# ablab/spades

Measured on NVIDIA H100. Metric: Mk-mers/s (extract+count+index) k=55, 150 bp reads, higher is better.
Workload: dtype u64

## Files before the change

spades_b200/csrc/mphf.cu:

```cuda
#include <math.h>

#include <algorithm>

#include "mphf_dev.cuh"

namespace sg {

template <int NW>
__global__ void mphf_insert_k(KeyTable t, const uint64_t *__restrict__ alive, uint64_t n, int level, MphfDev m, uint64_t level_start,
                              uint64_t *__restrict__ coll) {
    uint64_t i = (uint64_t)blockIdx.x * blockDim.x + threadIdx.x;
    if (i >= n) return;
    const int64_t ki = alive ? (int64_t)alive[i] : (int64_t)i;
    Kmer<NW> k = table_key<NW>(t, ki);
    const uint32_t b = kmer_bucket<NW>(k, m.B);
    uint64_t w;
    const uint64_t pos = level_pos<NW>(m, k, b, level, &w);
    const unsigned long long bit = 1ull << (pos & 63);
    unsigned long long old = atomicOr((unsigned long long *)&m.bits[w], bit);
    if (old & bit) atomicOr((unsigned long long *)&coll[w - level_start], bit);
}

__global__ void mphf_clear_k(uint64_t *__restrict__ bits, uint64_t *__restrict__ coll, uint64_t nwords) {
    uint64_t i = (uint64_t)blockIdx.x * blockDim.x + threadIdx.x;
    if (i >= nwords) return;
    uint64_t c = coll[i];
    if (c) { bits[i] &= ~c; coll[i] = 0; }
}

template <int NW>
__global__ void mphf_filter_k(KeyTable t, const uint64_t *__restrict__ alive, uint64_t n, int level, MphfDev m, uint64_t *__restrict__ next,
                              uint64_t cap, unsigned long long *__restrict__ next_n) {
    uint64_t i = (uint64_t)blockIdx.x * blockDim.x + threadIdx.x;
    bool keep = false;
    int64_t ki = 0;
    if (i < n) {
        ki = alive ? (int64_t)alive[i] : (int64_t)i;
        Kmer<NW> k = table_key<NW>(t, ki);
        const uint32_t b = kmer_bucket<NW>(k, m.B);
        uint64_t w;
        const uint64_t pos = level_pos<NW>(m, k, b, level, &w);
        keep = !((m.bits[w] >> (pos & 63)) & 1ull);
    }
    __shared__ unsigned s_warp[8];
    __shared__ unsigned long long s_base;
    const unsigned mask = __ballot_sync(0xffffffffu, keep);
    const int lane = threadIdx.x & 31, warp = threadIdx.x >> 5;
    if (lane == 0) s_warp[warp] = __popc(mask);
    __syncthreads();
    if (threadIdx.x == 0) {
        unsigned tot = 0;
        for (int w = 0; w < 8; ++w) { unsigned c = s_warp[w]; s_warp[w] = tot; tot += c; }
        s_base = tot ? atomicAdd(next_n, (unsigned long long)tot) : 0ull;
    }
    __syncthreads();
    if (keep) {
        const uint64_t slot = s_base + s_warp[warp] + __popc(mask & ((1u << lane) - 1));
        if (slot < cap) next[slot] = (uint64_t)ki;
    }
}

template <int NW>
__global__ void mphf_advance_k(KeyTable t, const uint64_t *__restrict__ alive, uint64_t n, int level, MphfDev m, uint64_t *__restrict__ next,
                               uint64_t cap, unsigned long long *__restrict__ next_n, int do_insert, uint64_t next_level_start,
                               uint64_t *__restrict__ coll) {
    uint64_t i = (uint64_t)blockIdx.x * blockDim.x + threadIdx.x;
    bool keep = false;
    int64_t ki = 0;
    if (i < n) {
        ki = alive ? (int64_t)alive[i] : (int64_t)i;
        Kmer<NW> k = table_key<NW>(t, ki);
        const uint32_t b = kmer_bucket<NW>(k, m.B);
        LevelHasher lh(xxh3_128<NW>(k));
        uint64_t h = 0;
        for (int l = 0; l <= level; ++l) h = lh.next();
        size_t p = (size_t)level * m.B + b;
        uint64_t pos = mulhi64(h, m.dom[p]);
        keep = !((m.bits[m.woff[p] + (pos >> 6)] >> (pos & 63)) & 1ull);
        if (keep && do_insert) {
            h = lh.next();
            p += m.B;
            pos = mulhi64(h, m.dom[p]);
            const uint64_t w = m.woff[p] + (pos >> 6);
            const unsigned long long bit = 1ull << (pos & 63);
            unsigned long long old = atomicOr((unsigned long long *)&m.bits[w], bit);
            if (old & bit) atomicOr((unsigned long long *)&coll[w - next_level_start], bit);
        }
    }
    __shared__ unsigned s_warp[8];
    __shared__ unsigned long long s_base;
    const unsigned mask = __ballot_sync(0xffffffffu, keep);
    const int lane = threadIdx.x & 31, warp = threadIdx.x >> 5;
    if (lane == 0) s_warp[warp] = __popc(mask);
    __syncthreads();
    if (threadIdx.x == 0) {
        unsigned tot = 0;
        for (int w = 0; w < 8; ++w) { unsigned c = s_warp[w]; s_warp[w] = tot; tot += c; }
        s_base = tot ? atomicAdd(next_n, (unsigned long long)tot) : 0ull;
    }
    __syncthreads();
    if (keep) {
        const uint64_t slot = s_base + s_warp[warp] + __popc(mask & ((1u << lane) - 1));
        if (slot < cap) next[slot] = (uint64_t)ki;
    }
}

__global__ void mphf_blockpop_k(const uint64_t *__restrict__ bits, uint64_t nblocks, uint32_t *__restrict__ pop) {
    uint64_t i = (uint64_t)blockIdx.x * blockDim.x + threadIdx.x;
    if (i >= nblocks) return;
    const ulonglong2 *p = reinterpret_cast<const ulonglong2 *>(bits + i * 8);
    uint32_t s = 0;
#pragma unroll
    for (int q = 0; q < 4; ++q) { ulonglong2 v = p[q]; s += __popcll(v.x) + __popcll(v.y); }
    pop[i] = s;
}

__global__ void mphf_piecebase_k(const uint64_t *__restrict__ gscan, const uint64_t *__restrict__ woff, uint32_t B, uint64_t total_blocks,
                                 uint64_t *__restrict__ piece_base, uint64_t *__restrict__ lastrank) {
    uint32_t b = blockIdx.x * blockDim.x + threadIdx.x;
    if (b >= B) return;
    uint64_t run = 0;
    for (int l = 0; l < kLevels; ++l) {
        const size_t p = (size_t)l * B + b;
        const uint64_t blk0 = woff[p] >> 3;
        const uint64_t blk1 = (p + 1 < (size_t)kLevels * B) ? (woff[p + 1] >> 3) : total_blocks;
        piece_base[p] = run;
        run += gscan[blk1] - gscan[blk0];
    }
    lastrank[b] = run;
}
__global__ void mphf_ranks_k(const uint64_t *__restrict__ gscan, const uint64_t *__restrict__ woff, const uint64_t *__restrict__ piece_base,
                             uint32_t npieces, uint64_t nblocks, uint64_t *__restrict__ ranks) {
    uint64_t i = (uint64_t)blockIdx.x * blockDim.x + threadIdx.x;
    if (i >= nblocks) return;
    uint32_t lo = 0, hi = npieces - 1;
    while (lo < hi) {
        uint32_t mid = (lo + hi + 1) >> 1;
        if ((woff[mid] >> 3) <= i) lo = mid; else hi = mid - 1;
    }
    ranks[i] = piece_base[lo] + gscan[i] - gscan[woff[lo] >> 3];
}

template <int NW>
__global__ void mphf_lookup_k(MphfDev m, const uint64_t *__restrict__ keys, uint64_t n, uint64_t *__restrict__ out) {
    uint64_t i = (uint64_t)blockIdx.x * blockDim.x + threadIdx.x;
    if (i >= n) return;
    Kmer<NW> k;
#pragma unroll
    for (int q = 0; q < NW; ++q) k.w[q] = keys[i * NW + q];
    out[i] = mphf_lookup_dev<NW>(m, k);
}

MphfDev mphf_dev(const Mphf *m) {
    MphfDev d;
    d.dom = m->d_dom.p; d.woff = m->d_woff.p; d.starts = m->d_starts.p; d.bits = m->bits.p; d.ranks = m->ranks.p; d.B = (uint32_t)m->B;
    return d;
}

template <int NW>
static void build_nw(Ctx *ctx, const KSet *ks, Mphf *m) {
    cudaStream_t st = ctx->stream;
    const int B = ks->B;
    const uint64_t n = (uint64_t)ks->n;
    m->dom.assign((size_t)kLevels * B, 0); m->nchar.assign((size_t)kLevels * B, 0); m->woff.assign((size_t)kLevels * B + 1, 0);
    std::vector<uint64_t> level_start(kLevels + 1, 0);
    {
        uint64_t off = 0;
        std::vector<double> pcol(B);
        std::vector<uint64_t> hd(B);
        for (int b = 0; b < B; ++b) {
            uint64_t nb = (uint64_t)ks->bsz[b];
            double gamma = 4.0;
            hd[b] = (uint64_t)ceil((double)nb * gamma);
            pcol[b] = nb ? 1.0 - pow(((gamma * (double)nb - 1) / (gamma * (double)nb)), (double)(nb - 1)) : 0.0;
        }
        for (int l = 0; l < kLevels; ++l) {
            level_start[l] = off;
            for (int b = 0; b < B; ++b) {
                const size_t p = (size_t)l * B + b;
                m->woff[p] = off;
                if (ks->bsz[b] == 0) { m->dom[p] = 64; m->nchar[p] = 0; continue; }
                uint64_t d = (((uint64_t)((double)hd[b] * pow(pcol[b], l)) + 63) / 64) * 64;
                if (d == 0) d = 64;
                m->dom[p] = d;
                m->nchar[p] = 1 + d / 64;
                off += ((m->nchar[p] + 7) / 8) * 8;
            }
        }
        level_start[kLevels] = off;
        m->woff[(size_t)kLevels * B] = off;
        m->total_words = off;
    }
    m->starts.assign(B + 1, 0);
    for (int b = 0; b < B; ++b) m->starts[b + 1] = (uint64_t)ks->bsz[b];
    for (int i = 1; i < B; ++i) m->starts[i] += m->starts[i - 1];
    m->bsz = ks->bsz;
    m->lastrank.assign(B, 0);
    const uint64_t total_words = m->total_words;
    const uint64_t nblocks = total_words / 8;
    m->bits.alloc(ctx, total_words + 8, true);
    m->ranks.alloc(ctx, nblocks + 1, true);
    m->d_dom.alloc(ctx, m->dom.size(), true); m->d_woff.alloc(ctx, m->woff.size(), true); m->d_starts.alloc(ctx, m->starts.size(), true);
    SG_CUDA(cudaMemsetAsync(m->bits.p, 0, m->bits.bytes(), st));
    SG_CUDA(cudaMemcpyAsync(m->d_dom.p, m->dom.data(), m->dom.size() * 8, cudaMemcpyHostToDevice, st));
    SG_CUDA(cudaMemcpyAsync(m->d_woff.p, m->woff.data(), m->woff.size() * 8, cudaMemcpyHostToDevice, st));
    SG_CUDA(cudaMemcpyAsync(m->d_starts.p, m->starts.data(), m->starts.size() * 8, cudaMemcpyHostToDevice, st));
    if (n == 0 || total_words == 0) { SG_CUDA(cudaStreamSynchronize(st)); return; }

    MphfDev md = mphf_dev(m);
    const uint64_t l0_words = level_start[1] - level_start[0];
    DArr<uint64_t> coll(ctx, l0_words + 8);
    SG_CUDA(cudaMemsetAsync(coll.p, 0, coll.bytes(), st));
    DArr<unsigned long long> d_cnt(ctx, 1);
    DArr<uint64_t> aliveA, aliveB;
    auto place = [&](const KeyTable &t, uint64_t n, int b_lo, int b_hi) {
        auto clear = [&](int l) {
            const uint64_t w0 = m->woff[(size_t)l * B + b_lo], nw = m->woff[(size_t)l * B + b_hi] - w0;
            mphf_clear_k<<<div_up((int64_t)nw, 256), 256, 0, st>>>(m->bits.p + w0, coll.p + (w0 - level_start[l]), nw);
            ctx->launches++;
        };
        const uint64_t *alive = nullptr;
        uint64_t n_alive = n;
        mphf_insert_k<NW><<<div_up((int64_t)n_alive, 256), 256, 0, st>>>(t, alive, n_alive, 0, md, level_start[0], coll.p);
        ctx->launches++;
        clear(0);
        for (int l = 0; l < kLevels - 1 && n_alive; ++l) {
            const bool last = (l == kLevels - 2);
            DArr<uint64_t> &next = (l & 1) ? aliveA : aliveB;
            uint64_t cap = (l == 0) ? n_alive / 2 + 1024 : n_alive;
            if (next.n < cap) next.alloc(ctx, cap);
            SG_CUDA(cudaMemsetAsync(d_cnt.p, 0, 8, st));
            mphf_advance_k<NW><<<div_up((int64_t)n_alive, 256), 256, 0, st>>>(t, alive, n_alive, l, md, next.p, (uint64_t)next.n, d_cnt.p,
                                                                             last ? 0 : 1, last ? 0 : level_start[l + 1], coll.p);
            ctx->launches++;
            if (!last) clear(l + 1);
            SG_CUDA(cudaGetLastError());
            unsigned long long c = 0;
            SG_CUDA(cudaMemcpyAsync(&c, d_cnt.p, 8, cudaMemcpyDeviceToHost, st));
            SG_CUDA(cudaStreamSynchronize(st));
            SG_CHECK(c <= next.n, 6, "internal: MPHF survivor list overflow");
            alive = next.p;
            n_alive = c;
        }
        SG_CHECK(n_alive == 0, 7, "MPHF: keys fell through all 24 bitset levels (reference would use its order-dependent fallback map); unsupported");
    };
    if (!ks->on_host) {
        place(make_table(ks), n, 0, B);
    } else {
        ChunkStager stage(ks, false);
        for (size_t c = 0; c < ks->chunks.size(); ++c) {
            const Chunk &ch = ks->chunks[c];
            const uint64_t *keys = nullptr;
            stage.acquire(c, &keys, nullptr);
            if (ch.n) {
                KeyTable t;
                t.nchunks = 1; t.first[0] = 0; t.first[1] = ch.n; t.keys[0] = keys;
                place(t, (uint64_t)ch.n, ch.b_lo, ch.b_hi);
            }
            stage.release(c);
        }
    }
    DArr<uint32_t> pop(ctx, nblocks + 1);
    DArr<uint64_t> gscan(ctx, nblocks + 1), piece_base(ctx, (size_t)kLevels * B), d_last(ctx, B);
    SG_CUDA(cudaMemsetAsync(pop.p + nblocks, 0, 4, st));
    mphf_blockpop_k<<<div_up((int64_t)nblocks, 256), 256, 0, st>>>(m->bits.p, nblocks, pop.p);
    ctx->launches++;
    exclusive_scan_u32_to_u64(ctx, pop.p, gscan.p, nblocks + 1);
    mphf_piecebase_k<<<div_up(B, 128), 128, 0, st>>>(gscan.p, m->d_woff.p, (uint32_t)B, nblocks, piece_base.p, d_last.p);
    mphf_ranks_k<<<div_up((int64_t)nblocks, 256), 256, 0, st>>>(gscan.p, m->d_woff.p, piece_base.p, (uint32_t)(kLevels * B), nblocks, m->ranks.p);
    ctx->launches += 2;
    SG_CUDA(cudaGetLastError());
    SG_CUDA(cudaMemcpyAsync(m->lastrank.data(), d_last.p, (size_t)B * 8, cudaMemcpyDeviceToHost, st));
    SG_CUDA(cudaStreamSynchronize(st));
    for (int b = 0; b < B; ++b) SG_CHECK(m->lastrank[b] == (uint64_t)ks->bsz[b], 6, "internal: MPHF is not minimal (rank total != bucket size)");
}

Mphf *mphf_build(Ctx *ctx, const KSet *ks) {
    Mphf *m = new Mphf();
    m->ctx = ctx; m->K = ks->K; m->nw = ks->nw; m->B = ks->B; m->n = ks->n;
    ctx->times.stage_h2d_bytes = 0;
    cudaEvent_t a, b;
    cudaEventCreate(&a); cudaEventCreate(&b);
    cudaEventRecord(a, ctx->stream);
    try {
        switch (ks->nw) {
            case 1: build_nw<1>(ctx, ks, m); break;
            case 2: build_nw<2>(ctx, ks, m); break;
            case 3: build_nw<3>(ctx, ks, m); break;
            default: build_nw<4>(ctx, ks, m); break;
        }
    } catch (...) { cudaEventDestroy(a); cudaEventDestroy(b); delete m; throw; }
    cudaEventRecord(b, ctx->stream);
    cudaEventSynchronize(b);
    float ms = 0; cudaEventElapsedTime(&ms, a, b);
    ctx->times.mphf += ms;
    cudaEventDestroy(a); cudaEventDestroy(b);
    return m;
}

struct SerPiece { uint64_t src_word; uint64_t dst_byte; uint64_t nwords; uint32_t from_ranks; uint32_t pad; };
struct SerPatch { uint64_t dst_byte; uint64_t value; uint32_t nbytes; uint32_t pad; };

__global__ void ser_pieces_k(const SerPiece *__restrict__ pieces, const uint64_t *__restrict__ bits, const uint64_t *__restrict__ ranks,
                             uint32_t *__restrict__ img32) {
    const SerPiece p = pieces[blockIdx.x];
    const uint64_t *src = (p.from_ranks ? ranks : bits) + p.src_word;
    uint32_t *dst = img32 + (p.dst_byte >> 2);
    for (uint64_t i = threadIdx.x; i < p.nwords; i += blockDim.x) {
        const uint64_t v = src[i];
        dst[2 * i] = (uint32_t)v;
        dst[2 * i + 1] = (uint32_t)(v >> 32);
    }
}
__global__ void ser_patches_k(const SerPatch *__restrict__ patches, uint64_t n, uint32_t *__restrict__ img32) {
    uint64_t i = (uint64_t)blockIdx.x * blockDim.x + threadIdx.x;
    if (i >= n) return;
    const SerPatch p = patches[i];
    img32[p.dst_byte >> 2] = (uint32_t)p.value;
    if (p.nbytes == 8) img32[(p.dst_byte >> 2) + 1] = (uint32_t)(p.value >> 32);
}

size_t mphf_serialized_size(const Mphf *m) {
    const int B = m->B;
    size_t total = 8;
    for (int b = 0; b < B; ++b) {
        total += 28 + 8;
        if (m->bsz[b])
            for (int l = 0; l < kLevels; ++l) {
                const size_t p = (size_t)l * B + b;
                total += 16 + 8 * m->nchar[p] + 8 + 8 * ((m->nchar[p] + 7) / 8);
            }
    }
    return total + 8 * ((size_t)B + 1);
}

void mphf_serialize_to(const Mphf *m, uint8_t *out, size_t cap) {
    Ctx *ctx = m->ctx;
    const int B = m->B;
    const size_t total = mphf_serialized_size(m);
    SG_CHECK(total <= cap, 2, "output buffer too small for the serialized index");
    std::vector<SerPiece> pieces;
    std::vector<SerPatch> patches;
    size_t pos = 0;
    auto patch = [&](uint64_t v, uint32_t nbytes) { patches.push_back(SerPatch{pos, v, nbytes, 0}); pos += nbytes; };
// ... 57 lines not shown
```

spades_b200/csrc/mphf_dev.cuh:

```cuda
#pragma once
#include "sgpu_internal.h"

namespace sg {

struct KeyTable {
    int nchunks;
    int64_t first[kMaxChunks + 1];
    const uint64_t *keys[kMaxChunks];
};

template <int NW>
__device__ __forceinline__ Kmer<NW> table_key(const KeyTable &t, int64_t i) {
    int c = 0, hi = t.nchunks - 1;
    while (c < hi) {
        const int mid = (c + hi + 1) >> 1;
        if (t.first[mid] <= i) c = mid; else hi = mid - 1;
    }
    const uint64_t *p = t.keys[c] + (i - t.first[c]) * NW;
    Kmer<NW> k;
#pragma unroll
    for (int q = 0; q < NW; ++q) k.w[q] = p[q];
    return k;
}

struct MphfDev {
    const uint64_t *dom;
    const uint64_t *woff;
    const uint64_t *starts;
    uint64_t *bits;
    const uint64_t *ranks;
    uint32_t B;
};

template <int NW>
__device__ __forceinline__ uint64_t level_pos(const MphfDev &m, const Kmer<NW> &k, uint32_t b, int level, uint64_t *word_index) {
    LevelHasher lh(xxh3_128<NW>(k));
    uint64_t h = 0;
    for (int l = 0; l <= level; ++l) h = lh.next();
    const uint64_t pos = mulhi64(h, m.dom[(size_t)level * m.B + b]);
    *word_index = m.woff[(size_t)level * m.B + b] + (pos >> 6);
    return pos;
}

template <int NW>
__device__ __forceinline__ uint64_t mphf_lookup_dev(const MphfDev &m, const Kmer<NW> &k) {
    const uint32_t b = kmer_bucket<NW>(k, m.B);
    LevelHasher lh(xxh3_128<NW>(k));
    for (int l = 0; l < kLevels - 1; ++l) {
        const uint64_t h = lh.next();
        const size_t p = (size_t)l * m.B + b;
        const uint64_t pos = mulhi64(h, m.dom[p]);
        const uint64_t wbase = m.woff[p];
        const uint64_t wi = pos >> 6;
        const uint64_t word = m.bits[wbase + wi];
        if ((word >> (pos & 63)) & 1ull) {
            uint64_t r = m.ranks[(wbase >> 3) + (pos >> 9)];
            for (uint64_t w = (pos >> 9) << 3; w < wi; ++w) r += __popcll(m.bits[wbase + w]);
            r += __popcll(word & ((1ull << (pos & 63)) - 1));
            return m.starts[b] + r;
        }
    }
    return ~0ull;
}


MphfDev mphf_dev(const Mphf *m);

inline KeyTable make_table(const KSet *ks) {
    SG_CHECK((int)ks->chunks.size() <= kMaxChunks, 6, "too many result chunks for the key table");
    KeyTable t;
    t.nchunks = (int)ks->chunks.size();
    for (int c = 0; c < t.nchunks; ++c) { t.first[c] = ks->chunks[c].first; t.keys[c] = ks->chunks[c].keys.p; }
    t.first[t.nchunks] = ks->n;
    if (t.nchunks == 0) { t.nchunks = 1; t.first[0] = 0; t.first[1] = 0; t.keys[0] = nullptr; }
    return t;
}

}
```

Before: 8693.

## Carry hasher state for surviving keys across MPHF levels instead of rehashing

The MPHF placement no longer reloads each surviving k-mer and recomputes xxh3 and the level-hash chain at every level. It now stores the hasher state (s0, s1) and the bucket id in survivor arrays and resumes from there. Bucket ids come from a binary search over the sorted bucket boundaries instead of rehashing, keys are read with streaming vectorized loads, and each thread handles four items in a grid-stride loop. Placement is also split into bucket ranges sized to the free device memory. In exchange, more bytes are written per survivor and the code is considerably more complex.

```diff
diff --git a/spades_b200/csrc/mphf.cu b/spades_b200/csrc/mphf.cu
--- a/spades_b200/csrc/mphf.cu
+++ b/spades_b200/csrc/mphf.cu
@@ -6,19 +6,198 @@
 
 namespace sg {
 
+static const int kPlaceThreads = 256, kPlaceU = 4, kPlaceTile = kPlaceThreads * kPlaceU, kPlaceCtasPerSm = 4;
 template <int NW>
-__global__ void mphf_insert_k(KeyTable t, const uint64_t *__restrict__ alive, uint64_t n, int level, MphfDev m, uint64_t level_start,
-                              uint64_t *__restrict__ coll) {
-    uint64_t i = (uint64_t)blockIdx.x * blockDim.x + threadIdx.x;
-    if (i >= n) return;
-    const int64_t ki = alive ? (int64_t)alive[i] : (int64_t)i;
-    Kmer<NW> k = table_key<NW>(t, ki);
-    const uint32_t b = kmer_bucket<NW>(k, m.B);
-    uint64_t w;
-    const uint64_t pos = level_pos<NW>(m, k, b, level, &w);
-    const unsigned long long bit = 1ull << (pos & 63);
-    unsigned long long old = atomicOr((unsigned long long *)&m.bits[w], bit);
-    if (old & bit) atomicOr((unsigned long long *)&coll[w - level_start], bit);
+constexpr int test0_ctas_per_sm() { return NW >= 4 ? 2 : NW >= 2 ? 3 : kPlaceCtasPerSm; }
+
+struct PlaceRange {
+    const uint64_t *bnd;
+    uint64_t base;
+    uint32_t b_lo, b_hi;
+};
+
+__device__ __forceinline__ uint32_t bucket_at(const uint64_t *__restrict__ bnd, uint32_t lo, uint32_t hi, uint64_t g) {
+    while (lo < hi) {
+        const uint32_t mid = (lo + hi + 1) >> 1;
+        if (__ldg(bnd + mid) <= g) lo = mid; else hi = mid - 1;
+    }
+    return lo;
+}
+
+template <int NW>
+__device__ __forceinline__ Kmer<NW> load_key_stream(const uint64_t *__restrict__ keys, uint64_t i) {
+    Kmer<NW> k;
+    const uint64_t *p = keys + i * NW;
+    if (NW % 2 == 0) {
+#pragma unroll
+        for (int q = 0; q < NW; q += 2) { const ulonglong2 v = __ldcs(reinterpret_cast<const ulonglong2 *>(p + q)); k.w[q] = v.x; k.w[q + 1] = v.y; }
+    } else {
+#pragma unroll
+        for (int q = 0; q < NW; ++q) k.w[q] = __ldcs(p + q);
+    }
+    return k;
+}
+
+__device__ __forceinline__ void level_insert(const MphfDev &m, const size_t (&p)[kPlaceU], const uint64_t (&h)[kPlaceU], unsigned todo,
+                                             uint64_t level_start, uint64_t *__restrict__ coll) {
+    uint64_t w[kPlaceU];
+    unsigned long long bit[kPlaceU], old[kPlaceU];
+#pragma unroll
+    for (int j = 0; j < kPlaceU; ++j) {
+        w[j] = 0; bit[j] = 0; old[j] = 0;
+        if ((todo >> j) & 1u) {
+            const uint64_t pos = mulhi64(h[j], __ldg(m.dom + p[j]));
+            w[j] = __ldg(m.woff + p[j]) + (pos >> 6);
+            bit[j] = 1ull << (pos & 63);
+            old[j] = atomicOr((unsigned long long *)&m.bits[w[j]], bit[j]);
+        }
+    }
+#pragma unroll
+    for (int j = 0; j < kPlaceU; ++j)
+        if (old[j] & bit[j]) atomicOr((unsigned long long *)&coll[w[j] - level_start], bit[j]);
+}
+
+__device__ __forceinline__ bool level_bit(const MphfDev &m, size_t p, uint64_t h) {
+    const uint64_t pos = mulhi64(h, __ldg(m.dom + p));
+    return (m.bits[__ldg(m.woff + p) + (pos >> 6)] >> (pos & 63)) & 1ull;
+}
+
+struct LevelStates {
+    uint64_t *s0, *s1;
+    uint32_t *b;
+};
+
+__device__ __forceinline__ void tile_buckets(const PlaceRange &r, uint64_t t0, uint64_t t1, uint32_t *lo, uint32_t *hi) {
+    *lo = bucket_at(r.bnd, r.b_lo, r.b_hi - 1, r.base + t0);
+    *hi = bucket_at(r.bnd, *lo, r.b_hi - 1, r.base + t1 - 1);
+}
+
+__device__ __forceinline__ void append_states(const uint64_t (&s0)[kPlaceU], const uint64_t (&s1)[kPlaceU], const uint32_t (&b)[kPlaceU], unsigned keep,
+                                              LevelStates out, uint64_t cap, unsigned long long *__restrict__ out_n) {
+    __shared__ unsigned s_warp[kPlaceThreads / 32];
+    __shared__ unsigned long long s_base;
+    const int lane = threadIdx.x & 31, warp = threadIdx.x >> 5;
+    const unsigned c = __popc(keep);
+    unsigned incl = c;
+#pragma unroll
+    for (int d = 1; d < 32; d <<= 1) { const unsigned v = __shfl_up_sync(0xffffffffu, incl, d); if (lane >= d) incl += v; }
+    if (lane == 31) s_warp[warp] = incl;
+    __syncthreads();
+    if (threadIdx.x == 0) {
+        unsigned tot = 0;
+#pragma unroll
+        for (int w = 0; w < kPlaceThreads / 32; ++w) { const unsigned v = s_warp[w]; s_warp[w] = tot; tot += v; }
+        s_base = tot ? atomicAdd(out_n, (unsigned long long)tot) : 0ull;
+    }
+    __syncthreads();
+    uint64_t slot = s_base + s_warp[warp] + (incl - c);
+#pragma unroll
+    for (int j = 0; j < kPlaceU; ++j)
+        if ((keep >> j) & 1u) {
+            if (slot < cap) { out.s0[slot] = s0[j]; out.s1[slot] = s1[j]; out.b[slot] = b[j]; }
+            ++slot;
+        }
+}
+
+template <int NW>
+__global__ void __launch_bounds__(kPlaceThreads, kPlaceCtasPerSm) mphf_insert0_k(const uint64_t *__restrict__ keys, uint64_t n, PlaceRange r, MphfDev m,
+                                                                uint64_t level_start, uint64_t *__restrict__ coll) {
+    for (uint64_t t0 = (uint64_t)blockIdx.x * kPlaceTile; t0 < n; t0 += (uint64_t)gridDim.x * kPlaceTile) {
+        const uint64_t t1 = min(t0 + (uint64_t)kPlaceTile, n);
+        uint32_t blo, bhi;
+        tile_buckets(r, t0, t1, &blo, &bhi);
+        Kmer<NW> k[kPlaceU];
+#pragma unroll
+        for (int j = 0; j < kPlaceU; ++j) {
+            const uint64_t i = t0 + (uint64_t)j * kPlaceThreads + threadIdx.x;
+            if (i < t1) k[j] = load_key_stream<NW>(keys, i);
+        }
+        size_t p[kPlaceU];
+        uint64_t h[kPlaceU];
+        unsigned todo = 0;
+#pragma unroll
+        for (int j = 0; j < kPlaceU; ++j) {
+            const uint64_t i = t0 + (uint64_t)j * kPlaceThreads + threadIdx.x;
+            p[j] = 0; h[j] = 0;
+            if (i < t1) { p[j] = bucket_at(r.bnd, blo, bhi, r.base + i); h[j] = xxh3_128<NW>(k[j]).hi; todo |= 1u << j; }
+        }
+        level_insert(m, p, h, todo, level_start, coll);
+    }
+}
+
+template <int NW>
+__global__ void __launch_bounds__(kPlaceThreads, test0_ctas_per_sm<NW>()) mphf_test0_k(const uint64_t *__restrict__ keys, uint64_t n, PlaceRange r, MphfDev m,
+                                                              LevelStates out, uint64_t cap, unsigned long long *__restrict__ out_n,
+                                                              uint64_t next_level_start, uint64_t *__restrict__ coll) {
+    for (uint64_t t0 = (uint64_t)blockIdx.x * kPlaceTile; t0 < n; t0 += (uint64_t)gridDim.x * kPlaceTile) {
+        const uint64_t t1 = min(t0 + (uint64_t)kPlaceTile, n);
+        uint32_t blo, bhi;
+        tile_buckets(r, t0, t1, &blo, &bhi);
+        Kmer<NW> k[kPlaceU];
+#pragma unroll
+        for (int j = 0; j < kPlaceU; ++j) {
+            const uint64_t i = t0 + (uint64_t)j * kPlaceThreads + threadIdx.x;
+            if (i < t1) k[j] = load_key_stream<NW>(keys, i);
+        }
+        uint64_t s0[kPlaceU], s1[kPlaceU];
+        uint32_t b[kPlaceU];
+        bool set[kPlaceU];
+#pragma unroll
+        for (int j = 0; j < kPlaceU; ++j) {
+            const uint64_t i = t0 + (uint64_t)j * kPlaceThreads + threadIdx.x;
+            set[j] = true;
+            if (i < t1) {
+                const Hash128 h = xxh3_128<NW>(k[j]);
+                s0[j] = h.hi; s1[j] = h.lo;
+                b[j] = bucket_at(r.bnd, blo, bhi, r.base + i);
+                set[j] = level_bit(m, b[j], s0[j]);
+            }
+        }
+        unsigned keep = 0;
+        size_t p[kPlaceU];
+#pragma unroll
+        for (int j = 0; j < kPlaceU; ++j) {
+            keep |= (set[j] ? 0u : 1u) << j;
+            p[j] = (size_t)m.B + b[j];
+        }
+        level_insert(m, p, s1, keep, next_level_start, coll);
+        append_states(s0, s1, b, keep, out, cap, out_n);
+    }
+}
+
+__global__ void __launch_bounds__(kPlaceThreads, kPlaceCtasPerSm) mphf_advance_k(LevelStates in, uint64_t n, int level, MphfDev m, LevelStates out, uint64_t cap,
+                                                                unsigned long long *__restrict__ out_n, int do_insert, uint64_t next_level_start,
+                                                                uint64_t *__restrict__ coll) {
+    for (uint64_t t0 = (uint64_t)blockIdx.x * kPlaceTile; t0 < n; t0 += (uint64_t)gridDim.x * kPlaceTile) {
+        const uint64_t t1 = min(t0 + (uint64_t)kPlaceTile, n);
+        uint64_t s0[kPlaceU], s1[kPlaceU];
+        uint32_t b[kPlaceU];
+#pragma unroll
+        for (int j = 0; j < kPlaceU; ++j) {
+            const uint64_t i = t0 + (uint64_t)j * kPlaceThreads + threadIdx.x;
+            if (i < t1) { s0[j] = __ldcs(in.s0 + i); s1[j] = __ldcs(in.s1 + i); b[j] = __ldcs(in.b + i); }
+        }
+        unsigned keep = 0;
+        size_t p[kPlaceU];
+        uint64_t h1[kPlaceU];
+#pragma unroll
+        for (int j = 0; j < kPlaceU; ++j) {
+            const uint64_t i = t0 + (uint64_t)j * kPlaceThreads + threadIdx.x;
+            p[j] = (size_t)(level + 1) * m.B + b[j]; h1[j] = 0;
+            if (i < t1) {
+                LevelHasher lh(Hash128{s1[j], s0[j]});
+                lh.level = level;
+                const uint64_t h = lh.next();
+                if (!level_bit(m, (size_t)level * m.B + b[j], h)) {
+                    keep |= 1u << j;
+                    s0[j] = lh.s0; s1[j] = lh.s1;
+                    h1[j] = lh.next();
+                }
+            }
+        }
+        if (do_insert) level_insert(m, p, h1, keep, next_level_start, coll);
+        append_states(s0, s1, b, keep, out, cap, out_n);
+    }
 }
 
 __global__ void mphf_clear_k(uint64_t *__restrict__ bits, uint64_t *__restrict__ coll, uint64_t nwords) {
@@ -26,83 +205,6 @@
     if (i >= nwords) return;
     uint64_t c = coll[i];
     if (c) { bits[i] &= ~c; coll[i] = 0; }
-}
-
-template <int NW>
-__global__ void mphf_filter_k(KeyTable t, const uint64_t *__restrict__ alive, uint64_t n, int level, MphfDev m, uint64_t *__restrict__ next,
-                              uint64_t cap, unsigned long long *__restrict__ next_n) {
-    uint64_t i = (uint64_t)blockIdx.x * blockDim.x + threadIdx.x;
-    bool keep = false;
-    int64_t ki = 0;
-    if (i < n) {
-        ki = alive ? (int64_t)alive[i] : (int64_t)i;
-        Kmer<NW> k = table_key<NW>(t, ki);
-        const uint32_t b = kmer_bucket<NW>(k, m.B);
-        uint64_t w;
-        const uint64_t pos = level_pos<NW>(m, k, b, level, &w);
-        keep = !((m.bits[w] >> (pos & 63)) & 1ull);
-    }
-    __shared__ unsigned s_warp[8];
-    __shared__ unsigned long long s_base;
-    const unsigned mask = __ballot_sync(0xffffffffu, keep);
-    const int lane = threadIdx.x & 31, warp = threadIdx.x >> 5;
-    if (lane == 0) s_warp[warp] = __popc(mask);
-    __syncthreads();
-    if (threadIdx.x == 0) {
-        unsigned tot = 0;
-        for (int w = 0; w < 8; ++w) { unsigned c = s_warp[w]; s_warp[w] = tot; tot += c; }
-        s_base = tot ? atomicAdd(next_n, (unsigned long long)tot) : 0ull;
-    }
-    __syncthreads();
-    if (keep) {
-        const uint64_t slot = s_base + s_warp[warp] + __popc(mask & ((1u << lane) - 1));
-        if (slot < cap) next[slot] = (uint64_t)ki;
-    }
-}
-
-template <int NW>
-__global__ void mphf_advance_k(KeyTable t, const uint64_t *__restrict__ alive, uint64_t n, int level, MphfDev m, uint64_t *__restrict__ next,
-                               uint64_t cap, unsigned long long *__restrict__ next_n, int do_insert, uint64_t next_level_start,
-                               uint64_t *__restrict__ coll) {
-    uint64_t i = (uint64_t)blockIdx.x * blockDim.x + threadIdx.x;
-    bool keep = false;
-    int64_t ki = 0;
-    if (i < n) {
-        ki = alive ? (int64_t)alive[i] : (int64_t)i;
-        Kmer<NW> k = table_key<NW>(t, ki);
-        const uint32_t b = kmer_bucket<NW>(k, m.B);
-        LevelHasher lh(xxh3_128<NW>(k));
-        uint64_t h = 0;
-        for (int l = 0; l <= level; ++l) h = lh.next();
-        size_t p = (size_t)level * m.B + b;
-        uint64_t pos = mulhi64(h, m.dom[p]);
-        keep = !((m.bits[m.woff[p] + (pos >> 6)] >> (pos & 63)) & 1ull);
-        if (keep && do_insert) {
-            h = lh.next();
-            p += m.B;
-            pos = mulhi64(h, m.dom[p]);
-            const uint64_t w = m.woff[p] + (pos >> 6);
-            const unsigned long long bit = 1ull << (pos & 63);
-            unsigned long long old = atomicOr((unsigned long long *)&m.bits[w], bit);
-            if (old & bit) atomicOr((unsigned long long *)&coll[w - next_level_start], bit);
-        }
-    }
-    __shared__ unsigned s_warp[8];
-    __shared__ unsigned long long s_base;
-    const unsigned mask = __ballot_sync(0xffffffffu, keep);
-    const int lane = threadIdx.x & 31, warp = threadIdx.x >> 5;
-    if (lane == 0) s_warp[warp] = __popc(mask);
-    __syncthreads();
-    if (threadIdx.x == 0) {
-        unsigned tot = 0;
-        for (int w = 0; w < 8; ++w) { unsigned c = s_warp[w]; s_warp[w] = tot; tot += c; }
-        s_base = tot ? atomicAdd(next_n, (unsigned long long)tot) : 0ull;
-    }
-    __syncthreads();
-    if (keep) {
-        const uint64_t slot = s_base + s_warp[warp] + __popc(mask & ((1u << lane) - 1));
-        if (slot < cap) next[slot] = (uint64_t)ki;
-    }
 }
 
 __global__ void mphf_blockpop_k(const uint64_t *__restrict__ bits, uint64_t nblocks, uint32_t *__restrict__ pop) {
@@ -208,55 +310,90 @@
     if (n == 0 || total_words == 0) { SG_CUDA(cudaStreamSynchronize(st)); return; }
 
     MphfDev md = mphf_dev(m);
-    const uint64_t l0_words = level_start[1] - level_start[0];
-    DArr<uint64_t> coll(ctx, l0_words + 8);
-    SG_CUDA(cudaMemsetAsync(coll.p, 0, coll.bytes(), st));
+    std::vector<uint64_t> bnd(B + 1, 0);
+    for (int b = 0; b < B; ++b) bnd[b + 1] = bnd[b] + (uint64_t)ks->bsz[b];
+    SG_CHECK(bnd[B] == n, 6, "internal: bucket sizes do not add up to the set size");
+    DArr<uint64_t> d_bnd(ctx, B + 1);
+    SG_CUDA(cudaMemcpyAsync(d_bnd.p, bnd.data(), (size_t)(B + 1) * 8, cudaMemcpyHostToDevice, st));
     DArr<unsigned long long> d_cnt(ctx, 1);
-    DArr<uint64_t> aliveA, aliveB;
-    auto place = [&](const KeyTable &t, uint64_t n, int b_lo, int b_hi) {
+    auto grid = [&](uint64_t items) { return (int)std::min<uint64_t>((uint64_t)INT32_MAX, (items + kPlaceTile - 1) / kPlaceTile); };
+    struct States {
+        DArr<uint64_t> s0, s1;
+        DArr<uint32_t> b;
+        void alloc(Ctx *c, uint64_t cap) { s0.alloc(c, cap); s1.alloc(c, cap); b.alloc(c, cap); }
+        LevelStates view() { return LevelStates{s0.p, s1.p, b.p}; }
+    };
+    auto place = [&](const uint64_t *keys, int b_lo, int b_hi) {
+        const uint64_t nr = bnd[b_hi] - bnd[b_lo];
+        if (nr == 0) return;
+        const PlaceRange r{d_bnd.p, bnd[b_lo], (uint32_t)b_lo, (uint32_t)b_hi};
+        auto w_at = [&](int l) { return m->woff[(size_t)l * B + b_lo]; };
+        auto nw_at = [&](int l) { return m->woff[(size_t)l * B + b_hi] - w_at(l); };
+        DArr<uint64_t> coll(ctx, nw_at(0) + 8);
+        SG_CUDA(cudaMemsetAsync(coll.p, 0, coll.bytes(), st));
         auto clear = [&](int l) {
-            const uint64_t w0 = m->woff[(size_t)l * B + b_lo], nw = m->woff[(size_t)l * B + b_hi] - w0;
-            mphf_clear_k<<<div_up((int64_t)nw, 256), 256, 0, st>>>(m->bits.p + w0, coll.p + (w0 - level_start[l]), nw);
+            mphf_clear_k<<<div_up((int64_t)nw_at(l), 256), 256, 0, st>>>(m->bits.p + w_at(l), coll.p, nw_at(l));
             ctx->launches++;
         };
-        const uint64_t *alive = nullptr;
-        uint64_t n_alive = n;
-        mphf_insert_k<NW><<<div_up((int64_t)n_alive, 256), 256, 0, st>>>(t, alive, n_alive, 0, md, level_start[0], coll.p);
+        mphf_insert0_k<NW><<<grid(nr), kPlaceThreads, 0, st>>>(keys, nr, r, md, w_at(0), coll.p);
         ctx->launches++;
         clear(0);
-        for (int l = 0; l < kLevels - 1 && n_alive; ++l) {
-            const bool last = (l == kLevels - 2);
-            DArr<uint64_t> &next = (l & 1) ? aliveA : aliveB;
-            uint64_t cap = (l == 0) ? n_alive / 2 + 1024 : n_alive;
-            if (next.n < cap) next.alloc(ctx, cap);
-            SG_CUDA(cudaMemsetAsync(d_cnt.p, 0, 8, st));
-            mphf_advance_k<NW><<<div_up((int64_t)n_alive, 256), 256, 0, st>>>(t, alive, n_alive, l, md, next.p, (uint64_t)next.n, d_cnt.p,
-                                                                             last ? 0 : 1, last ? 0 : level_start[l + 1], coll.p);
-            ctx->launches++;
-            if (!last) clear(l + 1);
+        States A, Bs;
+        A.alloc(ctx, nr / 2 + 1024);
+        uint64_t cap = A.s0.n;
+        SG_CUDA(cudaMemsetAsync(d_cnt.p, 0, 8, st));
+        mphf_test0_k<NW><<<grid(nr), kPlaceThreads, 0, st>>>(keys, nr, r, md, A.view(), cap, d_cnt.p, w_at(1), coll.p);
+        ctx->launches++;
+        clear(1);
+        States *cur = &A, *nxt = &Bs;
+        uint64_t n_alive = 0;
+        for (int l = 1;; ++l) {
             SG_CUDA(cudaGetLastError());
             unsigned long long c = 0;
             SG_CUDA(cudaMemcpyAsync(&c, d_cnt.p, 8, cudaMemcpyDeviceToHost, st));
             SG_CUDA(cudaStreamSynchronize(st));
-            SG_CHECK(c <= next.n, 6, "internal: MPHF survivor list overflow");
-            alive = next.p;
+            SG_CHECK(c <= cap, 6, "internal: MPHF survivor list overflow");
             n_alive = c;
+            if (n_alive == 0 || l == kLevels - 1) break;
+            const bool last = (l == kLevels - 2);
+            if (nxt->s0.n < n_alive) nxt->alloc(ctx, n_alive);
+            cap = nxt->s0.n;
+            SG_CUDA(cudaMemsetAsync(d_cnt.p, 0, 8, st));
+            mphf_advance_k<<<grid(n_alive), kPlaceThreads, 0, st>>>(cur->view(), n_alive, l, md, nxt->view(), cap, d_cnt.p, last ? 0 : 1,
+                                                                    last ? 0 : w_at(l + 1), coll.p);
+            ctx->launches++;
+            if (!last) clear(l + 1);
+            std::swap(cur, nxt);
         }
         SG_CHECK(n_alive == 0, 7, "MPHF: keys fell through all 24 bitset levels (reference would use its order-dependent fallback map); unsupported");
     };
+    uint64_t knob_keys = 0;
+    if (const char *e = getenv("SGPU_MPHF_RANGE_KEYS")) knob_keys = strtoull(e, nullptr, 10);
+    auto place_chunk = [&](const uint64_t *keys, int64_t n_keys, int b_lo, int b_hi) {
+        SG_CHECK(bnd[b_hi] - bnd[b_lo] == (uint64_t)n_keys, 6, "internal: a chunk's keys are not its buckets' keys");
+        const size_t room = ctx->free_bytes();
+        auto scratch = [&](int lo, int hi) {
+            const uint64_t k = bnd[hi] - bnd[lo];
+            return (double)(8 * (m->woff[hi] - m->woff[lo] + 8)) + 40.0 * (double)(k / 2 + 1024);
+        };
+        int lo = b_lo;
+        while (lo < b_hi) {
+            int hi = lo + 1;
+            while (hi < b_hi && scratch(lo, hi + 1) <= (double)room && (knob_keys == 0 || bnd[hi + 1] - bnd[lo] <= knob_keys)) ++hi;
+            place(keys + (bnd[lo] - bnd[b_lo]) * NW, lo, hi);
+            lo = hi;
+        }
+    };
     if (!ks->on_host) {
-        place(make_table(ks), n, 0, B);
+        for (const Chunk &ch : ks->chunks)
+            if (ch.n) place_chunk(ch.keys.p, ch.n, ch.b_lo, ch.b_hi);
     } else {
         ChunkStager stage(ks, false);
         for (size_t c = 0; c < ks->chunks.size(); ++c) {
             const Chunk &ch = ks->chunks[c];
             const uint64_t *keys = nullptr;
             stage.acquire(c, &keys, nullptr);
-            if (ch.n) {
-                KeyTable t;
-                t.nchunks = 1; t.first[0] = 0; t.first[1] = ch.n; t.keys[0] = keys;
-                place(t, (uint64_t)ch.n, ch.b_lo, ch.b_hi);
-            }
+            if (ch.n) place_chunk(keys, ch.n, ch.b_lo, ch.b_hi);
             stage.release(c);
         }
     }
diff --git a/spades_b200/csrc/mphf_dev.cuh b/spades_b200/csrc/mphf_dev.cuh
--- a/spades_b200/csrc/mphf_dev.cuh
+++ b/spades_b200/csrc/mphf_dev.cuh
@@ -2,26 +2,6 @@
 #include "sgpu_internal.h"
 
 namespace sg {
-
-struct KeyTable {
-    int nchunks;
-    int64_t first[kMaxChunks + 1];
-    const uint64_t *keys[kMaxChunks];
-};
-
-template <int NW>
-__device__ __forceinline__ Kmer<NW> table_key(const KeyTable &t, int64_t i) {
-    int c = 0, hi = t.nchunks - 1;
-    while (c < hi) {
-        const int mid = (c + hi + 1) >> 1;
-        if (t.first[mid] <= i) c = mid; else hi = mid - 1;
-    }
-    const uint64_t *p = t.keys[c] + (i - t.first[c]) * NW;
-    Kmer<NW> k;
-#pragma unroll
-    for (int q = 0; q < NW; ++q) k.w[q] = p[q];
-    return k;
-}
 
 struct MphfDev {
     const uint64_t *dom;
@@ -31,16 +11,6 @@
     const uint64_t *ranks;
     uint32_t B;
 };
-
-template <int NW>
-__device__ __forceinline__ uint64_t level_pos(const MphfDev &m, const Kmer<NW> &k, uint32_t b, int level, uint64_t *word_index) {
-    LevelHasher lh(xxh3_128<NW>(k));
-    uint64_t h = 0;
-    for (int l = 0; l <= level; ++l) h = lh.next();
-    const uint64_t pos = mulhi64(h, m.dom[(size_t)level * m.B + b]);
-    *word_index = m.woff[(size_t)level * m.B + b] + (pos >> 6);
-    return pos;
-}
 
 template <int NW>
 __device__ __forceinline__ uint64_t mphf_lookup_dev(const MphfDev &m, const Kmer<NW> &k) {
@@ -66,14 +36,4 @@
 
 MphfDev mphf_dev(const Mphf *m);
 
-inline KeyTable make_table(const KSet *ks) {
-    SG_CHECK((int)ks->chunks.size() <= kMaxChunks, 6, "too many result chunks for the key table");
-    KeyTable t;
-    t.nchunks = (int)ks->chunks.size();
-    for (int c = 0; c < t.nchunks; ++c) { t.first[c] = ks->chunks[c].first; t.keys[c] = ks->chunks[c].keys.p; }
-    t.first[t.nchunks] = ks->n;
-    if (t.nchunks == 0) { t.nchunks = 1; t.first[0] = 0; t.first[1] = 0; t.keys[0] = nullptr; }
-    return t;
 }
-
-}
```

Measured after the change: 8834, median of 6. 1.02x the previous value.

## Carry hash state in survivor lists and tile MPHF build by bucket

Applied to the files above, without the earlier changes.

The MPHF build now stores each surviving key's hash-generator state and bucket, instead of its key index. Later levels therefore skip re-reading the k-mer, re-hashing it and replaying the hasher from level zero. Level 0 is processed per bucket tile, so dom/woff are loaded once per block, and keys are streamed with vectorised cache-streaming loads at two keys per thread. The clear kernel now also counts placed bits, which lets the host know the expected survivor count. This adds survivor buffers of roughly 2.5 words per key and relies on the LevelHasher state layout (level, s0, s1) being resumable.

```diff
diff --git a/spades_b200/csrc/mphf.cu b/spades_b200/csrc/mphf.cu
--- a/spades_b200/csrc/mphf.cu
+++ b/spades_b200/csrc/mphf.cu
@@ -6,102 +6,230 @@
 
 namespace sg {
 
+static const int kSweepThreads = 256;
+static const int kKeysPerThread = 2;
+static const int kTileKeys = kSweepThreads * kKeysPerThread;
+
+struct TileMap {
+    const uint64_t *tile_first;
+    uint64_t ntiles;
+    uint64_t n;
+    uint64_t kbase;
+    int b_lo, b_hi;
+};
+struct Tile { const uint64_t *keys; uint32_t cnt; uint32_t b; };
+
 template <int NW>
-__global__ void mphf_insert_k(KeyTable t, const uint64_t *__restrict__ alive, uint64_t n, int level, MphfDev m, uint64_t level_start,
-                              uint64_t *__restrict__ coll) {
-    uint64_t i = (uint64_t)blockIdx.x * blockDim.x + threadIdx.x;
-    if (i >= n) return;
-    const int64_t ki = alive ? (int64_t)alive[i] : (int64_t)i;
-    Kmer<NW> k = table_key<NW>(t, ki);
-    const uint32_t b = kmer_bucket<NW>(k, m.B);
-    uint64_t w;
-    const uint64_t pos = level_pos<NW>(m, k, b, level, &w);
-    const unsigned long long bit = 1ull << (pos & 63);
-    unsigned long long old = atomicOr((unsigned long long *)&m.bits[w], bit);
-    if (old & bit) atomicOr((unsigned long long *)&coll[w - level_start], bit);
-}
-
-__global__ void mphf_clear_k(uint64_t *__restrict__ bits, uint64_t *__restrict__ coll, uint64_t nwords) {
-    uint64_t i = (uint64_t)blockIdx.x * blockDim.x + threadIdx.x;
-    if (i >= nwords) return;
-    uint64_t c = coll[i];
-    if (c) { bits[i] &= ~c; coll[i] = 0; }
+__device__ __forceinline__ Tile tile_at(const KeyTable &t, const TileMap &tm, const MphfDev &m, uint64_t tile) {
+    int lo = 0, hi = tm.b_hi - tm.b_lo - 1;
+    while (lo < hi) {
+        const int mid = (lo + hi + 1) >> 1;
+        if (tm.tile_first[mid] <= tile) lo = mid; else hi = mid - 1;
+    }
+    const uint32_t b = (uint32_t)(tm.b_lo + lo);
+    const uint64_t kbeg = m.starts[b] - tm.kbase;
+    const uint64_t kend = ((int)b + 1 < tm.b_hi) ? m.starts[b + 1] - tm.kbase : tm.n;
+    const uint64_t i0 = kbeg + (tile - tm.tile_first[lo]) * kTileKeys;
+    Tile r;
+    r.b = b;
+    r.cnt = (uint32_t)min((uint64_t)kTileKeys, kend - i0);
+    r.keys = table_chunk_key(t, (int64_t)i0, NW);
+    return r;
 }
 
 template <int NW>
-__global__ void mphf_filter_k(KeyTable t, const uint64_t *__restrict__ alive, uint64_t n, int level, MphfDev m, uint64_t *__restrict__ next,
-                              uint64_t cap, unsigned long long *__restrict__ next_n) {
-    uint64_t i = (uint64_t)blockIdx.x * blockDim.x + threadIdx.x;
-    bool keep = false;
-    int64_t ki = 0;
-    if (i < n) {
-        ki = alive ? (int64_t)alive[i] : (int64_t)i;
-        Kmer<NW> k = table_key<NW>(t, ki);
-        const uint32_t b = kmer_bucket<NW>(k, m.B);
-        uint64_t w;
-        const uint64_t pos = level_pos<NW>(m, k, b, level, &w);
-        keep = !((m.bits[w] >> (pos & 63)) & 1ull);
-    }
-    __shared__ unsigned s_warp[8];
+__device__ __forceinline__ Kmer<NW> stream_key(const uint64_t *p) {
+    Kmer<NW> k;
+    if (NW % 2 == 0) {
+#pragma unroll
+        for (int q = 0; q < NW / 2; ++q) {
+            const ulonglong2 v = __ldcs(reinterpret_cast<const ulonglong2 *>(p) + q);
+            k.w[2 * q] = v.x; k.w[2 * q + 1] = v.y;
+        }
+    } else {
+#pragma unroll
+        for (int q = 0; q < NW; ++q) k.w[q] = __ldcs(reinterpret_cast<const unsigned long long *>(p) + q);
+    }
+    return k;
+}
+
+template <int U>
+__device__ __forceinline__ void insert_bits(uint64_t *bits, uint64_t *coll, uint64_t level_start, const uint64_t (&w)[U], const uint64_t (&pos)[U],
+                                            const bool (&on)[U]) {
+    unsigned long long old[U];
+#pragma unroll
+    for (int u = 0; u < U; ++u)
+        if (on[u]) old[u] = atomicOr((unsigned long long *)&bits[w[u]], 1ull << (pos[u] & 63));
+#pragma unroll
+    for (int u = 0; u < U; ++u)
+        if (on[u] && (old[u] & (1ull << (pos[u] & 63)))) atomicOr((unsigned long long *)&coll[w[u] - level_start], 1ull << (pos[u] & 63));
+}
+
+struct SurvDev {
+    uint64_t *s0, *s1;
+    uint32_t *b;
+};
+
+template <int U>
+__device__ __forceinline__ void block_append(const bool (&keep)[U], unsigned long long *next_n, uint64_t (&slot)[U]) {
+    __shared__ unsigned s_warp[kSweepThreads / 32];
     __shared__ unsigned long long s_base;
-    const unsigned mask = __ballot_sync(0xffffffffu, keep);
     const int lane = threadIdx.x & 31, warp = threadIdx.x >> 5;
-    if (lane == 0) s_warp[warp] = __popc(mask);
+    unsigned run = 0, off[U];
+#pragma unroll
+    for (int u = 0; u < U; ++u) {
+        const unsigned mask = __ballot_sync(0xffffffffu, keep[u]);
+        off[u] = run + __popc(mask & ((1u << lane) - 1));
+        run += __popc(mask);
+    }
+    if (lane == 0) s_warp[warp] = run;
     __syncthreads();
     if (threadIdx.x == 0) {
         unsigned tot = 0;
-        for (int w = 0; w < 8; ++w) { unsigned c = s_warp[w]; s_warp[w] = tot; tot += c; }
+        for (int w = 0; w < kSweepThreads / 32; ++w) { const unsigned c = s_warp[w]; s_warp[w] = tot; tot += c; }
         s_base = tot ? atomicAdd(next_n, (unsigned long long)tot) : 0ull;
     }
     __syncthreads();
-    if (keep) {
-        const uint64_t slot = s_base + s_warp[warp] + __popc(mask & ((1u << lane) - 1));
-        if (slot < cap) next[slot] = (uint64_t)ki;
-    }
+    const uint64_t base = s_base + s_warp[warp];
+#pragma unroll
+    for (int u = 0; u < U; ++u) slot[u] = base + off[u];
 }
 
 template <int NW>
-__global__ void mphf_advance_k(KeyTable t, const uint64_t *__restrict__ alive, uint64_t n, int level, MphfDev m, uint64_t *__restrict__ next,
-                               uint64_t cap, unsigned long long *__restrict__ next_n, int do_insert, uint64_t next_level_start,
-                               uint64_t *__restrict__ coll) {
-    uint64_t i = (uint64_t)blockIdx.x * blockDim.x + threadIdx.x;
-    bool keep = false;
-    int64_t ki = 0;
-    if (i < n) {
-        ki = alive ? (int64_t)alive[i] : (int64_t)i;
-        Kmer<NW> k = table_key<NW>(t, ki);
-        const uint32_t b = kmer_bucket<NW>(k, m.B);
-        LevelHasher lh(xxh3_128<NW>(k));
-        uint64_t h = 0;
-        for (int l = 0; l <= level; ++l) h = lh.next();
-        size_t p = (size_t)level * m.B + b;
-        uint64_t pos = mulhi64(h, m.dom[p]);
-        keep = !((m.bits[m.woff[p] + (pos >> 6)] >> (pos & 63)) & 1ull);
-        if (keep && do_insert) {
-            h = lh.next();
-            p += m.B;
-            pos = mulhi64(h, m.dom[p]);
-            const uint64_t w = m.woff[p] + (pos >> 6);
-            const unsigned long long bit = 1ull << (pos & 63);
-            unsigned long long old = atomicOr((unsigned long long *)&m.bits[w], bit);
-            if (old & bit) atomicOr((unsigned long long *)&coll[w - next_level_start], bit);
-        }
-    }
-    __shared__ unsigned s_warp[8];
-    __shared__ unsigned long long s_base;
-    const unsigned mask = __ballot_sync(0xffffffffu, keep);
-    const int lane = threadIdx.x & 31, warp = threadIdx.x >> 5;
-    if (lane == 0) s_warp[warp] = __popc(mask);
+__global__ void __launch_bounds__(kSweepThreads) mphf_insert0_k(KeyTable t, TileMap tm, MphfDev m, uint64_t *__restrict__ coll) {
+    constexpr int U = kKeysPerThread;
+    {
+        const Tile tl = tile_at<NW>(t, tm, m, blockIdx.x);
+        const uint64_t dom = m.dom[tl.b], woff = m.woff[tl.b];
+        Kmer<NW> k[U];
+        bool on[U];
+#pragma unroll
+        for (int u = 0; u < U; ++u) {
+            const uint32_t i = threadIdx.x + u * kSweepThreads;
+            on[u] = i < tl.cnt;
+            if (on[u]) k[u] = stream_key<NW>(tl.keys + (size_t)i * NW);
+        }
+        uint64_t pos[U], w[U];
+#pragma unroll
+        for (int u = 0; u < U; ++u) {
+            pos[u] = on[u] ? mulhi64(xxh3_128<NW>(k[u]).hi, dom) : 0;
+            w[u] = woff + (pos[u] >> 6);
+        }
+        insert_bits<U>(m.bits, coll, 0, w, pos, on);
+    }
+}
+
+template <int NW>
+__global__ void __launch_bounds__(kSweepThreads) mphf_advance0_k(KeyTable t, TileMap tm, MphfDev m, SurvDev next, uint64_t cap,
+                                                                 unsigned long long *__restrict__ next_n, uint64_t level1_start,
+                                                                 uint64_t *__restrict__ coll1) {
+    constexpr int U = kKeysPerThread;
+    {
+        const Tile tl = tile_at<NW>(t, tm, m, blockIdx.x);
+        const uint64_t dom0 = m.dom[tl.b], woff0 = m.woff[tl.b], dom1 = m.dom[m.B + tl.b], woff1 = m.woff[m.B + tl.b];
+        Kmer<NW> k[U];
+        bool on[U];
+#pragma unroll
+        for (int u = 0; u < U; ++u) {
+            const uint32_t i = threadIdx.x + u * kSweepThreads;
+            on[u] = i < tl.cnt;
+            if (on[u]) k[u] = stream_key<NW>(tl.keys + (size_t)i * NW);
+        }
+        Hash128 h[U];
+        uint64_t word[U];
+#pragma unroll
+        for (int u = 0; u < U; ++u) {
+            h[u] = on[u] ? xxh3_128<NW>(k[u]) : Hash128{0, 0};
+            if (on[u]) word[u] = m.bits[woff0 + (mulhi64(h[u].hi, dom0) >> 6)];
+        }
+        bool keep[U];
+        uint64_t pos[U], w[U];
+#pragma unroll
+        for (int u = 0; u < U; ++u) {
+            keep[u] = on[u] && !((word[u] >> (mulhi64(h[u].hi, dom0) & 63)) & 1ull);
+            pos[u] = mulhi64(h[u].lo, dom1);
+            w[u] = woff1 + (pos[u] >> 6);
+        }
+        insert_bits<U>(m.bits, coll1, level1_start, w, pos, keep);
+        uint64_t slot[U];
+        block_append<U>(keep, next_n, slot);
+#pragma unroll
+        for (int u = 0; u < U; ++u)
+            if (keep[u] && slot[u] < cap) { next.s0[slot[u]] = h[u].hi; next.s1[slot[u]] = h[u].lo; next.b[slot[u]] = tl.b; }
+    }
+}
+
+__global__ void __launch_bounds__(kSweepThreads) mphf_advance_k(SurvDev cur, uint64_t n, int level, MphfDev m, SurvDev next, uint64_t cap,
+                                                                unsigned long long *__restrict__ next_n, uint64_t next_level_start,
+                                                                uint64_t *__restrict__ coll1) {
+    constexpr int U = kKeysPerThread;
+    {
+        const uint64_t base = (uint64_t)blockIdx.x * kTileKeys;
+        bool on[U];
+        uint64_t s0[U], s1[U];
+        uint32_t b[U];
+#pragma unroll
+        for (int u = 0; u < U; ++u) {
+            const uint64_t i = base + threadIdx.x + u * kSweepThreads;
+            on[u] = i < n;
+            s0[u] = on[u] ? __ldcs((const unsigned long long *)cur.s0 + i) : 0;
+            s1[u] = on[u] ? __ldcs((const unsigned long long *)cur.s1 + i) : 0;
+            b[u] = on[u] ? __ldcs(cur.b + i) : 0;
+        }
+        uint64_t pos[U], word[U];
+#pragma unroll
+        for (int u = 0; u < U; ++u) {
+            LevelHasher lh(Hash128{s1[u], s0[u]});
+            lh.level = level;
+            const size_t p = (size_t)level * m.B + b[u];
+            pos[u] = mulhi64(lh.next(), m.dom[p]);
+            s0[u] = lh.s0; s1[u] = lh.s1;
+            if (on[u]) word[u] = m.bits[m.woff[p] + (pos[u] >> 6)];
+        }
+        bool keep[U];
+        uint64_t w[U];
+#pragma unroll
+        for (int u = 0; u < U; ++u) {
+            keep[u] = on[u] && !((word[u] >> (pos[u] & 63)) & 1ull);
+            LevelHasher lh(Hash128{s1[u], s0[u]});
+            lh.level = level + 1;
+            const size_t p = (size_t)(level + 1) * m.B + b[u];
+            pos[u] = mulhi64(lh.next(), m.dom[p]);
+            w[u] = m.woff[p] + (pos[u] >> 6);
+        }
+        insert_bits<U>(m.bits, coll1, next_level_start, w, pos, keep);
+        uint64_t slot[U];
+        block_append<U>(keep, next_n, slot);
+#pragma unroll
+        for (int u = 0; u < U; ++u)
+            if (keep[u] && slot[u] < cap) { next.s0[slot[u]] = s0[u]; next.s1[slot[u]] = s1[u]; next.b[slot[u]] = b[u]; }
+    }
+}
+
+__global__ void __launch_bounds__(kSweepThreads) mphf_clear_k(uint64_t *__restrict__ bits, uint64_t *__restrict__ coll, uint64_t nwords,
+                                                              unsigned long long *__restrict__ placed) {
+    unsigned long long cnt = 0;
+    ulonglong2 *b2 = reinterpret_cast<ulonglong2 *>(bits);
+    ulonglong2 *c2 = reinterpret_cast<ulonglong2 *>(coll);
+    for (uint64_t i = (uint64_t)blockIdx.x * blockDim.x + threadIdx.x; i < nwords / 2; i += (uint64_t)gridDim.x * blockDim.x) {
+        const ulonglong2 c = c2[i];
+        ulonglong2 v = b2[i];
+        if (c.x | c.y) {
+            v.x &= ~c.x; v.y &= ~c.y;
+            b2[i] = v;
+            c2[i] = make_ulonglong2(0, 0);
+        }
+        cnt += __popcll(v.x) + __popcll(v.y);
+    }
+    __shared__ unsigned long long s_cnt[kSweepThreads / 32];
+#pragma unroll
+    for (int o = 16; o; o >>= 1) cnt += __shfl_xor_sync(0xffffffffu, cnt, o);
+    if ((threadIdx.x & 31) == 0) s_cnt[threadIdx.x >> 5] = cnt;
     __syncthreads();
     if (threadIdx.x == 0) {
-        unsigned tot = 0;
-        for (int w = 0; w < 8; ++w) { unsigned c = s_warp[w]; s_warp[w] = tot; tot += c; }
-        s_base = tot ? atomicAdd(next_n, (unsigned long long)tot) : 0ull;
-    }
-    __syncthreads();
-    if (keep) {
-        const uint64_t slot = s_base + s_warp[warp] + __popc(mask & ((1u << lane) - 1));
-        if (slot < cap) next[slot] = (uint64_t)ki;
+        unsigned long long tot = 0;
+        for (int w = 0; w < kSweepThreads / 32; ++w) tot += s_cnt[w];
+        if (tot) atomicAdd(placed, tot);
     }
 }
 
@@ -211,38 +339,63 @@
     const uint64_t l0_words = level_start[1] - level_start[0];
     DArr<uint64_t> coll(ctx, l0_words + 8);
     SG_CUDA(cudaMemsetAsync(coll.p, 0, coll.bytes(), st));
-    DArr<unsigned long long> d_cnt(ctx, 1);
-    DArr<uint64_t> aliveA, aliveB;
+    DArr<unsigned long long> d_cnt(ctx, 2);
+    DArr<uint64_t> d_tiles(ctx, (size_t)B + 1);
+    std::vector<uint64_t> h_tiles((size_t)B + 1);
+    struct Survivors {
+        DArr<uint64_t> buf;
+        uint64_t cap = 0;
+        void reserve(Ctx *c, uint64_t n) { if (n > cap) { buf.alloc(c, 2 * n + (n + 1) / 2); cap = n; } }
+        SurvDev dev() const { return SurvDev{buf.p, buf.p + cap, reinterpret_cast<uint32_t *>(buf.p + 2 * cap)}; }
+    } surv[2];
     auto place = [&](const KeyTable &t, uint64_t n, int b_lo, int b_hi) {
+        uint64_t placed = 0;
         auto clear = [&](int l) {
             const uint64_t w0 = m->woff[(size_t)l * B + b_lo], nw = m->woff[(size_t)l * B + b_hi] - w0;
-            mphf_clear_k<<<div_up((int64_t)nw, 256), 256, 0, st>>>(m->bits.p + w0, coll.p + (w0 - level_start[l]), nw);
-            ctx->launches++;
+            SG_CUDA(cudaMemsetAsync(d_cnt.p + 1, 0, 8, st));
+            if (nw) {
+                mphf_clear_k<<<std::min(div_up((int64_t)nw / 2, kSweepThreads), ctx->num_sms * 8), kSweepThreads, 0, st>>>(m->bits.p + w0, coll.p + (w0 - level_start[l]), nw, d_cnt.p + 1);
+                ctx->launches++;
+            }
         };
-        const uint64_t *alive = nullptr;
-        uint64_t n_alive = n;
-        mphf_insert_k<NW><<<div_up((int64_t)n_alive, 256), 256, 0, st>>>(t, alive, n_alive, 0, md, level_start[0], coll.p);
+        auto sync_counts = [&](unsigned long long *appended) {
+            SG_CUDA(cudaGetLastError());
+            unsigned long long c[2] = {0, 0};
+            SG_CUDA(cudaMemcpyAsync(c, d_cnt.p, 16, cudaMemcpyDeviceToHost, st));
+            SG_CUDA(cudaStreamSynchronize(st));
+            if (appended) *appended = c[0];
+            placed = c[1];
+        };
+        h_tiles[0] = 0;
+        for (int b = b_lo; b < b_hi; ++b) h_tiles[b - b_lo + 1] = h_tiles[b - b_lo] + div_up(ks->bsz[b], kTileKeys);
+        TileMap tm;
+        tm.tile_first = d_tiles.p; tm.ntiles = h_tiles[b_hi - b_lo]; tm.n = n; tm.kbase = m->starts[b_lo]; tm.b_lo = b_lo; tm.b_hi = b_hi;
+        SG_CUDA(cudaMemcpyAsync(d_tiles.p, h_tiles.data(), (size_t)(b_hi - b_lo + 1) * 8, cudaMemcpyHostToDevice, st));
+        mphf_insert0_k<NW><<<(unsigned)tm.ntiles, kSweepThreads, 0, st>>>(t, tm, md, coll.p);
         ctx->launches++;
         clear(0);
-        for (int l = 0; l < kLevels - 1 && n_alive; ++l) {
-            const bool last = (l == kLevels - 2);
-            DArr<uint64_t> &next = (l & 1) ? aliveA : aliveB;
-            uint64_t cap = (l == 0) ? n_alive / 2 + 1024 : n_alive;
-            if (next.n < cap) next.alloc(ctx, cap);
+        sync_counts(nullptr);
+        uint64_t n_alive = n;
+        for (int l = 0;; ++l) {
+            const uint64_t expect = n_alive - placed;
+            if (expect == 0) break;
+            SG_CHECK(l + 2 < kLevels, 7, "MPHF: keys fell through all 24 bitset levels (reference would use its order-dependent fallback map); unsupported");
+            Survivors &cur = surv[l & 1], &next = surv[(l + 1) & 1];
+            next.reserve(ctx, expect);
             SG_CUDA(cudaMemsetAsync(d_cnt.p, 0, 8, st));
-            mphf_advance_k<NW><<<div_up((int64_t)n_alive, 256), 256, 0, st>>>(t, alive, n_alive, l, md, next.p, (uint64_t)next.n, d_cnt.p,
-                                                                             last ? 0 : 1, last ? 0 : level_start[l + 1], coll.p);
+            if (l == 0)
+                mphf_advance0_k<NW><<<(unsigned)tm.ntiles, kSweepThreads, 0, st>>>(t, tm, md, next.dev(), next.cap, d_cnt.p, level_start[1],
+                                                                                          coll.p);
+            else
+                mphf_advance_k<<<div_up((int64_t)n_alive, kTileKeys), kSweepThreads, 0, st>>>(cur.dev(), n_alive, l, md, next.dev(),
+                                                                                                               next.cap, d_cnt.p, level_start[l + 1], coll.p);
             ctx->launches++;
-            if (!last) clear(l + 1);
-            SG_CUDA(cudaGetLastError());
-            unsigned long long c = 0;
-            SG_CUDA(cudaMemcpyAsync(&c, d_cnt.p, 8, cudaMemcpyDeviceToHost, st));
-            SG_CUDA(cudaStreamSynchronize(st));
-            SG_CHECK(c <= next.n, 6, "internal: MPHF survivor list overflow");
-            alive = next.p;
-            n_alive = c;
-        }
-        SG_CHECK(n_alive == 0, 7, "MPHF: keys fell through all 24 bitset levels (reference would use its order-dependent fallback map); unsupported");
+            clear(l + 1);
+            unsigned long long appended = 0;
+            sync_counts(&appended);
+            SG_CHECK(appended == expect, 6, "internal: MPHF survivors appended differ from the keys left unplaced");
+            n_alive = expect;
+        }
     };
     if (!ks->on_host) {
         place(make_table(ks), n, 0, B);
@@ -260,6 +413,8 @@
             stage.release(c);
         }
     }
+    for (Survivors &v : surv) v.buf.release();
+    coll.release();
     DArr<uint32_t> pop(ctx, nblocks + 1);
     DArr<uint64_t> gscan(ctx, nblocks + 1), piece_base(ctx, (size_t)kLevels * B), d_last(ctx, B);
     SG_CUDA(cudaMemsetAsync(pop.p + nblocks, 0, 4, st));
diff --git a/spades_b200/csrc/mphf_dev.cuh b/spades_b200/csrc/mphf_dev.cuh
--- a/spades_b200/csrc/mphf_dev.cuh
+++ b/spades_b200/csrc/mphf_dev.cuh
@@ -9,18 +9,13 @@
     const uint64_t *keys[kMaxChunks];
 };
 
-template <int NW>
-__device__ __forceinline__ Kmer<NW> table_key(const KeyTable &t, int64_t i) {
+__device__ __forceinline__ const uint64_t *table_chunk_key(const KeyTable &t, int64_t i, int nw) {
     int c = 0, hi = t.nchunks - 1;
     while (c < hi) {
         const int mid = (c + hi + 1) >> 1;
         if (t.first[mid] <= i) c = mid; else hi = mid - 1;
     }
-    const uint64_t *p = t.keys[c] + (i - t.first[c]) * NW;
-    Kmer<NW> k;
-#pragma unroll
-    for (int q = 0; q < NW; ++q) k.w[q] = p[q];
-    return k;
+    return t.keys[c] + (i - t.first[c]) * nw;
 }
 
 struct MphfDev {
@@ -31,16 +26,6 @@
     const uint64_t *ranks;
     uint32_t B;
 };
-
-template <int NW>
-__device__ __forceinline__ uint64_t level_pos(const MphfDev &m, const Kmer<NW> &k, uint32_t b, int level, uint64_t *word_index) {
-    LevelHasher lh(xxh3_128<NW>(k));
-    uint64_t h = 0;
-    for (int l = 0; l <= level; ++l) h = lh.next();
-    const uint64_t pos = mulhi64(h, m.dom[(size_t)level * m.B + b]);
-    *word_index = m.woff[(size_t)level * m.B + b] + (pos >> 6);
-    return pos;
-}
 
 template <int NW>
 __device__ __forceinline__ uint64_t mphf_lookup_dev(const MphfDev &m, const Kmer<NW> &k) {
```

Result: faster. 8711 before, 8888 after (median of 6 runs) (+2.0%).
